# q-optimize/c3

Measured on AMD Instinct MI355X. Metric: full-gate propagators/s, higher is better.
Workload: dtype c128

## Files before the change

c3_amd/csrc/c3p_smalld.hip:

```cpp
#include <type_traits>

#include <cstdlib>
#include "c3p_common.h"
#include "c3p_kernels.h"
#include "c3p_smalld.h"

#ifdef C3P_SMALLD_PART
#define C3P_SMALLD_HAS(p) (C3P_SMALLD_PART == (p))
#else
#define C3P_SMALLD_HAS(p) 1
#endif

extern __shared__ __attribute__((aligned(16))) double c3p_sd_lds[];

namespace {

template <int D>
struct SD {
  static constexpr int NBI = (D + 1) / 2;
  static constexpr int NJ = (D + 3) / 4;
  static constexpr int W = 4 * NJ + 1;
  static constexpr int MAT = 4 * NBI * W;
  static constexpr int IMG = ((MAT - 12 + 31) / 32) * 32 + 12;
};
// ... 575 lines not shown
#pragma unroll
    for (int I = 0; I < NC; ++I)
#pragma unroll
      for (int J = 0; J < NC; ++J) {
        T1[I][J] = Cc.vr[I] * Ur.rc[J];
        T2[I][J] = Sc.vr[I] * Ui.rc[J];
        T3[I][J] = dv[I] * us[J];
      }
  }
  double tr[NC], ti[NC], ar[NC], ai[NC];
#pragma unroll
  for (int J = 0; J < NC; ++J) {
    tr[J] = Cc.vr[0] * Ur.m[0][J];
    ti[J] = Cc.vr[0] * Ui.m[0][J];
#pragma unroll
    for (int K = 1; K < NC; ++K) {
      tr[J] = fma(Cc.vr[K], Ur.m[K][J], tr[J]);
      ti[J] = fma(Cc.vr[K], Ui.m[K][J], ti[J]);
    }
#pragma unroll
    for (int K = 0; K < NC; ++K) {
      tr[J] = fma(Sc.vr[K], Ui.m[K][J], tr[J]);
      ti[J] = fma(-Sc.vr[K], Ur.m[K][J], ti[J]);
    }
    ar[J] = fma(Sc.s, Ui.rc[J], Cc.s * Ur.rc[J]);
    ai[J] = fma(-Sc.s, Ur.rc[J], Cc.s * Ui.rc[J]);
  }
  double Pn[NC];
#pragma unroll
  for (int I = 0; I < NC; ++I) Pn[I] = fma(Sc.vr[I], Qs, Cc.vr[I] * Ub.Ps);
  double ts = Cc.vr[0] * Ub.Pc[0];
#pragma unroll
  for (int K = 1; K < NC; ++K) ts = fma(Cc.vr[K], Ub.Pc[K], ts);
#pragma unroll
  for (int K = 0; K < NC; ++K) ts = fma(Sc.vr[K], Qc[K], ts);
  const double es = fma(Sc.s, Qs, Cc.s * Ub.Ps);
#pragma unroll
  for (int K = 0; K < NC; ++K)
#pragma unroll
    for (int I = 0; I < NC; ++I) {
      Pn[I] = mfma4(Cc.m[K][I], Ub.Pc[K], Pn[I]);
#pragma unroll
      for (int J = 0; J < NC; ++J) {
        T1[I][J] = mfma4(Cc.m[K][I], Ur.m[K][J], T1[I][J]);
        T2[I][J] = mfma4(Sc.m[K][I], Ui.m[K][J], T2[I][J]);
        T3[I][J] = mfma4(Dm[K][I], Us[K][J], T3[I][J]);
      }
      Pn[I] = mfma4(Sc.m[K][I], Qc[K], Pn[I]);
    }
#pragma unroll
  for (int I = 0; I < NC; ++I) {
    Ur.rc[I] = mfma4(1.0, tr[I], ar[I]);
    Ui.rc[I] = mfma4(1.0, ti[I], ai[I]);
  }
  Ub.Ps = mfma4(1.0, ts, es);
#pragma unroll
  for (int I = 0; I < NC; ++I) Ub.Pc[I] = Pn[I];
#pragma unroll
  for (int I = 0; I < NC; ++I)
#pragma unroll
    for (int J = 0; J < NC; ++J) {
      Ur.m[I][J] = T1[I][J] + T2[I][J];
      Ui.m[I][J] = (T3[I][J] - T1[I][J]) + T2[I][J];
    }
}

__device__ __forceinline__ void plan_q4(double nrm, int& r, int& s) {
  const double th[5] = {4.0e-4, 5.45e-2, 3.18e-1, 8.16e-1, 1.49};
  int best_r = 5, best_s = 0, best_cost = 1 << 30;
#pragma unroll
  for (int i = 0; i < 5; ++i) {
    int si = c3p_squarings(nrm, th[i]);
    const int cost = i + si;
    if (cost < best_cost || (cost == best_cost && si <= best_s)) {
      best_cost = cost;
      best_r = i + 1;
      best_s = si;
    }
  }
  r = best_r;
  s = best_s;
}

template <int D>
__device__ __forceinline__ void row_phase_factors(const double* row_phase, const LanePos& lp, double (&pc)[SD<D>::NBI],
                                                  double (&ps)[SD<D>::NBI]) {
#pragma unroll
  for (int I = 0; I < SD<D>::NBI; ++I) {
    const int row = 2 * I + (lp.r >> 1);
    pc[I] = 1.0, ps[I] = 0.0;
    if (row_phase != nullptr && row < D) sincos(row_phase[row], &ps[I], &pc[I]);
  }
}

template <int D>
__device__ __forceinline__ void scale_rows(const double (&zh)[SD<D>::NBI][SD<D>::NJ], const double (&pr)[SD<D>::NBI],
                                           const double (&pi)[SD<D>::NBI], const LanePos& lp,
                                           double (&out)[SD<D>::NBI][SD<D>::NJ]) {
  using C = SD<D>;
  double oth[C::NBI][C::NJ];
#pragma unroll
  for (int I = 0; I < C::NBI; ++I)
#pragma unroll
    for (int J = 0; J < C::NJ; ++J) oth[I][J] = __shfl_xor(zh[I][J], 16);
#pragma unroll
  for (int I = 0; I < C::NBI; ++I)
#pragma unroll
    for (int J = 0; J < C::NJ; ++J)
      out[I][J] = (lp.r & 1) ? fma(pr[I], zh[I][J], pi[I] * oth[I][J]) : fma(pr[I], zh[I][J], -pi[I] * oth[I][J]);
}

template <int D, bool WRITE_THROUGH = false>
__device__ __forceinline__ void store_plain(const double (&zh)[SD<D>::NBI][SD<D>::NJ], double* dst,
                                            double sr, double si, const double* row_phase,
                                            const LanePos& lp, bool active, const double* pre_c = nullptr,
                                            const double* pre_s = nullptr) {
  using C = SD<D>;
  double pr[C::NBI], pi[C::NBI];
#pragma unroll
  for (int I = 0; I < C::NBI; ++I) {
    const int row = 2 * I + (lp.r >> 1);
    pr[I] = sr, pi[I] = si;
    if (pre_c != nullptr) {
      pr[I] = sr * pre_c[I] - si * pre_s[I];
      pi[I] = sr * pre_s[I] + si * pre_c[I];
    } else if (row_phase != nullptr && row < D) {
      double sn, cs;
      sincos(row_phase[row], &sn, &cs);
      pr[I] = sr * cs - si * sn;
      pi[I] = sr * sn + si * cs;
    }
  }
  double outv[C::NBI][C::NJ];
  scale_rows<D>(zh, pr, pi, lp, outv);
#pragma unroll
  for (int I = 0; I < C::NBI; ++I) {
    const int row = 2 * I + (lp.r >> 1);
#pragma unroll
    for (int J = 0; J < C::NJ; ++J) {
      const int col = 4 * J + lp.c;
      if (active && row < D && col < D) {
        double* p = dst + (row * D + col) * 2 + (lp.r & 1);
        if constexpr (WRITE_THROUGH) {
          __hip_atomic_store(reinterpret_cast<unsigned long long*>(p), (unsigned long long)__double_as_longlong(outv[I][J]),
                             __ATOMIC_RELAXED, __HIP_MEMORY_SCOPE_AGENT);
        } else {
          *p = outv[I][J];
        }
      }
    }
  }
}

__device__ __forceinline__ double wave_sum64(double v) {
#pragma unroll
  for (int o = 32; o > 0; o >>= 1) v += __shfl_xor(v, o);
  return v;
}
__device__ __forceinline__ double wave_max64(double v) {
#pragma unroll
  for (int o = 32; o > 0; o >>= 1) v = fmax(v, __shfl_xor(v, o));
  return v;
}

constexpr int SD_CSW = 16;

template <int D>
__device__ __forceinline__ double sd_colsum(const double* g, int j) {
  constexpr int W = SD<D>::W;
  double cs = 0.0;
  if (j < D) {
    double ar[D], ai[D];
#pragma unroll
    for (int i = 0; i < D; ++i) ar[i] = g[(2 * i) * W + j], ai[i] = g[(2 * i + 1) * W + j];
#pragma unroll
    for (int i = 0; i < D; ++i) cs += sqrt(fma(ar[i], ar[i], ai[i] * ai[i]));
  }
  return cs;
}

template <int D>
__device__ __forceinline__ void sd_colsums(const double* tab, int K, double* csb, int lane, int first = 0, int step = 1) {
  constexpr int MAT = SD<D>::MAT;
  for (int t0 = first; t0 <= K; t0 += 4 * step) {
    const int ti = t0 + (lane >> 4) * step;
    if (ti <= K) csb[ti * SD_CSW + (lane & 15)] = sd_colsum<D>(tab + ti * (MAT + 4), lane & 15);
  }
}

template <class F>
__device__ __forceinline__ double c3p_sd_segment_norm(const double* csb, int K, int idx16, F&& maxk) {
  double v = csb[idx16];
  for (int k = 0; k < K; ++k) v = fma(maxk(k), csb[(k + 1) * SD_CSW + idx16], v);
  v = fmax(v, __shfl_xor(v, 1));
  v = fmax(v, __shfl_xor(v, 2));
  v = fmax(v, __shfl_xor(v, 16));
  v = fmax(v, __shfl_xor(v, 32));
  return v;
}

template <int D>
__device__ __forceinline__ void build_tables(const SmallArgs& A, int sample, double* tab, double* csb, int lane, int first = 0, int step = 1) {
  using C = SD<D>;
  constexpr int MAT = C::MAT, W = C::W;
  constexpr int NE = (D * D + 63) / 64;
  for (int ti = first; ti <= A.K; ti += step) {
    double* out = tab + ti * (MAT + 4);
    const cplx* h = (ti == 0) ? A.h0 + (long)sample * A.h0_bstride
                              : A.hks + (long)sample * A.hks_bstride + (long)(ti - 1) * D * D;
    for (int e = lane; e < MAT; e += 64) out[e] = 0.0;
    double gr[NE], gi[NE];
    double tim = 0.0;
#pragma unroll
    for (int q = 0; q < NE; ++q) {
      const int e = lane + 64 * q;
      gr[q] = gi[q] = 0.0;
      if (e < D * D) {
        const cplx x = h[e];
        gr[q] = x.y * A.dt;
        gi[q] = -x.x * A.dt;
        if (e / D == e % D) tim += gi[q];
      }
    }
    const double mur = 0.0, mui = wave_sum64(tim) / D;
    wave_sync();
    double remax = 0.0;
#pragma unroll
    for (int q = 0; q < NE; ++q) {
      const int e = lane + 64 * q;
      if (e < D * D) {
        const int i = e / D, j = e - i * D;
        if (i == j) {
          gr[q] -= mur;
          gi[q] -= mui;
        }
        out[(2 * i) * W + j] = gr[q];
        out[(2 * i + 1) * W + j] = gi[q];
        remax = fmax(remax, fabs(gr[q]));
      }
    }
    wave_sync();
    const double cs = sd_colsum<D>(out, lane);
    if (lane < SD_CSW) csb[ti * SD_CSW + lane] = cs;
    const double nrm = wave_max64(cs);
    double asym = 0.0, rsk = 0.0;
#pragma unroll
    for (int q = 0; q < NE; ++q) {
      const int e = lane + 64 * q;
      if (e < D * D) {
        const int i = e / D, j = e - i * D;
        asym = fmax(asym, fabs(gi[q] - out[(2 * j + 1) * W + i]));
        rsk = fmax(rsk, fabs(gr[q] + out[(2 * j) * W + i]));
      }
    }
    asym = wave_max64(asym);
    rsk = wave_max64(rsk);
    if (asym > 1e-14 * nrm) remax = fmax(remax, asym);
    remax = wave_max64(remax);
    if (remax > 0.0 && fmax(asym, rsk) <= 1e-14 * nrm) remax = -remax;
    if (lane == 0) {
      out[MAT + 0] = mur;
      out[MAT + 1] = mui;
      out[MAT + 2] = nrm;
      out[MAT + 3] = remax;
    }
  }
  wave_sync();
}

template <int D, bool GIVEN, bool DUS, bool XG = false, bool MW = false, bool SPLIT = false>
__global__ void __launch_bounds__((MW ? 512 : 64), 2) smalld_chain_kernel(SmallArgs A) {
  using C = SD<D>;
  constexpr int NBI = C::NBI, NJ = C::NJ, W = C::W, MAT = C::MAT, IMG = C::IMG;
  const int lane = MW ? (threadIdx.x & 63) : threadIdx.x;
  const int wv = MW ? __builtin_amdgcn_readfirstlane(threadIdx.x >> 6) : 0;
  const int nwv = MW ? (int)(blockDim.x >> 6) : 1;
#ifdef C3P_SD_TIMING
  long long tk0 = wall_clock64(), tk1 = 0, tk2 = 0, tk3 = 0, tk4 = 0, tk5 = 0, tk6 = 0, tk7 = 0, tk8 = 0, tk9 = 0, tkl = 0, tka = 0, tkb = 0;
#define SD_TICK(v) v = wall_clock64()
#else
#define SD_TICK(v)
#endif
  LanePos lp;
  lp.r = lane >> 4;
  lp.b = (lane >> 2) & 3;
  lp.c = lane & 3;
  lp.idx16 = lp.r * 4 + lp.c;
  const int K = A.K;
  double* tab = c3p_sd_lds;
  const int SG = ((K + ((SPLIT && K > 0) ? 1 : 0)) * A.Lmax) | 1;
  double* img = tab + ((GIVEN || XG) ? 0 : (1 + K) * (MAT + 4)) + wv * (4 * IMG + 4 * SG);
  double* sg = img + 4 * IMG;
  double* csb = (!MW && (1 + K) * SD_CSW <= 4 * IMG) ? img : tab + (1 + K) * (MAT + 4) + nwv * (4 * IMG + 4 * SG);

  long lblock = blockIdx.x;
  if constexpr (MW)
    lblock = (long)blockIdx.x * nwv + wv;
  else if ((gridDim.x & 7) == 0)
    lblock = (long)(blockIdx.x & 7) * (gridDim.x >> 3) + (blockIdx.x >> 3);
  const long chain = lblock * 4 + lp.b;
  const long nchains = (long)A.B * A.S;
  const bool valid = chain < nchains;
  const long cc = valid ? chain : nchains - 1;
  const int sample = (int)(cc / A.S);
  const int seg = (int)(cc - (long)sample * A.S);
  int n0 = (int)(((long)seg * A.N) / A.S);
  int n1 = (int)(((long)(seg + 1) * A.N) / A.S);
  int len, tmax;
  auto split_segments = [&](int seg_long) {
    if (MW && seg_long > 0) {
      const int h = A.S >> 1;
      const long rest = (long)A.N - (long)h * seg_long;
      n0 = seg < h ? seg * seg_long : h * seg_long + (int)(((long)(seg - h) * rest) / h);
      n1 = seg + 1 <= h ? (seg + 1) * seg_long : h * seg_long + (int)(((long)(seg + 1 - h) * rest) / h);
    }
    len = n1 - n0;
    tmax = A.Lmax;
    if (MW && seg_long > 0) {
      int m = len;
      m = max(m, __shfl_xor(m, 4));
      m = max(m, __shfl_xor(m, 8));
      tmax = __builtin_amdgcn_readfirstlane(m);
    }
  };
  split_segments(A.seg_long);

  const int woff = lp.b * IMG + lp.r * W + lp.c;
  const int roff = lp.b * IMG + (2 * (lp.c >> 1) + ((lp.c ^ lp.r) & 1)) * W + (lp.r >> 1);
  const unsigned negmask = (((lp.c & 1) == 0) && ((lp.r & 1) == 1)) ? 0x80000000u : 0u;
  const int toff = lp.r * W + lp.c;
  const int ddelta = (lp.r & 1) ? 1000 : ((lp.r >> 1) - lp.c);
  const int rhalf = lp.r >> 1;

  double U[NBI][NJ];
  double mus_r = 0.0, mus_i = 0.0;
  bool img_holds_U = false;

  if constexpr (GIVEN) {
    const double* base = reinterpret_cast<const double*>(A.mats) + ((long)sample * A.N + n0) * D * D * 2;
    for (int t = 0; t < tmax; ++t) {
      const bool act = valid && t < len;
      double P[NBI][NJ];
      const double* src = base + (long)(act ? t : 0) * D * D * 2;
#pragma unroll
      for (int I = 0; I < NBI; ++I)
#pragma unroll
        for (int J = 0; J < NJ; ++J) {
          const int row = 2 * I + (lp.r >> 1), col = 4 * J + lp.c;
          P[I][J] = (act && row < D && col < D) ? src[(row * D + col) * 2 + (lp.r & 1)] : 0.0;
        }
      if (t == 0) {
#pragma unroll
        for (int I = 0; I < NBI; ++I)
#pragma unroll
          for (int J = 0; J < NJ; ++J) U[I][J] = P[I][J];
      } else {
        double acc[NBI][NJ];
#pragma unroll
        for (int I = 0; I < NBI; ++I)
#pragma unroll
          for (int J = 0; J < NJ; ++J) acc[I][J] = 0.0;
        if (A.right_order) {
          write_image<D>(U, img, woff);
          mm_img<D>(img, roff, negmask, P, acc);
        } else {
          write_image<D>(P, img, woff);
          mm_img<D>(img, roff, negmask, U, acc);
        }
#pragma unroll
        for (int I = 0; I < NBI; ++I)
#pragma unroll
          for (int J = 0; J < NJ; ++J) U[I][J] = act ? acc[I][J] : U[I][J];
      }
    }
  } else {
    double nrm = 0.0;
    if constexpr (XG) {
      const double* mt = A.meta + ((long)sample * A.N + n0) * 4;
      for (int t = lp.idx16; t < A.Lmax; t += 16)
        if (valid && t < len) nrm = fmax(nrm, mt[(long)t * 4 + 2]);
      nrm = fmax(nrm, __shfl_xor(nrm, 1));
      nrm = fmax(nrm, __shfl_xor(nrm, 2));
      nrm = fmax(nrm, __shfl_xor(nrm, 16));
      nrm = fmax(nrm, __shfl_xor(nrm, 32));
    } else {
    constexpr int PF_K = 2, PF_T = 3;
    const bool prefetch = MW && A.inline_tables && K <= PF_K && A.Lmax <= 16 * PF_T;
    double pre[PF_K][PF_T];
    if (prefetch) {
#pragma unroll
      for (int k = 0; k < PF_K; ++k)
#pragma unroll
        for (int i = 0; i < PF_T; ++i) {
          const int t = lp.idx16 + 16 * i;
          const double* sk = A.signals + ((long)sample * K + (k < K ? k : 0)) * A.N + n0;
          pre[k][i] = (k < K && valid && t < len) ? sk[t] : 0.0;
        }
    }
    if (A.inline_tables) {
      build_tables<D>(A, __builtin_amdgcn_readfirstlane(sample), tab, csb, lane, wv, nwv);
    } else {
      const double* gt0 = A.tables + (long)(A.tab_per_sample ? sample : 0) * (1 + K) * (MAT + 4);
      for (int e = (MW ? (int)threadIdx.x : lane); e < (1 + K) * (MAT + 4); e += 64 * nwv) tab[e] = gt0[e];
      __syncthreads();
      sd_colsums<D>(tab, K, csb, lane, wv, nwv);
    }
    if constexpr (!MW) __syncthreads();
    auto seg_max = [&](int k, bool from_lds) {
      const double* s = A.signals + ((long)sample * K + k) * A.N + n0;
      double cmax = 0.0;
      for (int t = lp.idx16; t < A.Lmax; t += 16) {
        double v;
        if (from_lds) {
          v = sg[lp.b * SG + k * A.Lmax + t];
        } else {
          v = (valid && t < len) ? s[t] : 0.0;
          sg[lp.b * SG + k * A.Lmax + t] = v;
        }
        cmax = fmax(cmax, fabs(v));
      }
      cmax = fmax(cmax, __shfl_xor(cmax, 1));
      cmax = fmax(cmax, __shfl_xor(cmax, 2));
      cmax = fmax(cmax, __shfl_xor(cmax, 16));
      cmax = fmax(cmax, __shfl_xor(cmax, 32));
      return cmax;
    };
    SD_TICK(tk8);
    if constexpr (MW) {
      if (prefetch) {
#pragma unroll
        for (int k = 0; k < PF_K; ++k)
#pragma unroll
          for (int i = 0; i < PF_T; ++i) {
            const int t = lp.idx16 + 16 * i;
            if (k < K && t < A.Lmax) sg[lp.b * SG + k * A.Lmax + t] = pre[k][i];
          }
      } else {
        for (int k = 0; k < K; ++k) (void)seg_max(k, false);
      }
      SD_TICK(tk9);
      __syncthreads();
      if (A.seg_long_c > 0 && A.seg_long_c != A.seg_long) {
        bool re = (A.mode == C3P_MODE_UNITARY);
        for (int k = 0; k <= K; ++k) re = re && (tab[k * (MAT + 4) + MAT + 3] == 0.0);
        if (__builtin_amdgcn_readfirstlane((int)re) == 0) {
          wave_sync();
          split_segments(A.seg_long_c);
          for (int k = 0; k < K; ++k) (void)seg_max(k, false);
          wave_sync();
        }
      }
    }
    nrm = c3p_sd_segment_norm(csb, K, lp.idx16, [&](int k) { return seg_max(k, MW); });
    }
    nrm = fmax(nrm, __shfl_xor(nrm, 4));
    nrm = fmax(nrm, __shfl_xor(nrm, 8));
    nrm = readfirstlane_f64(nrm);
    bool realH = !XG && (A.mode == C3P_MODE_UNITARY);
    if constexpr (!XG)
      for (int k = 0; k <= K; ++k) realH = realH && (tab[k * (MAT + 4) + MAT + 3] == 0.0);
    realH = __builtin_amdgcn_readfirstlane((int)realH) != 0;
    MfmaPlan plan = {0, 0, 0};
    int t18n = 0;
    if (!realH) {
      bool normalG = !XG && (A.mode == C3P_MODE_UNITARY) && !(A.no_t18n & 1);
      if constexpr (!XG)
        for (int k = 0; k <= K; ++k) normalG = normalG && (tab[k * (MAT + 4) + MAT + 3] <= 0.0);
      t18n = __builtin_amdgcn_readfirstlane((int)normalG);
      plan = c3p_pick_plan_mfma(nrm, t18n ? C3P_T18N_THETA : C3P_T18_THETA, t18n != 0 && !(A.no_t18n & 2));
    }
    const int pr = __builtin_amdgcn_readfirstlane(plan.r);
    const int ps = __builtin_amdgcn_readfirstlane(plan.s);
    const int t18 = __builtin_amdgcn_readfirstlane(plan.t18);
    const double scale = ldexp(1.0, -ps);
    __syncthreads();
    SD_TICK(tk1);

    if (realH) {
      constexpr int NB = RD<D>::NB;
      typedef double RMat[NB][NB];
      const int ps_r = __builtin_amdgcn_readfirstlane(c3p_squarings(nrm, C3P_MM8_THETA));
      const double rscale = ldexp(1.0, -ps_r);
      const int swap_lane = 16 * lp.c + 4 * lp.b + lp.r;
      const int tail_lane = 16 * lp.c + 4 * lp.b;
      const int row0_lane = 4 * lp.b + lp.c;
      RMat Ur, Ui;
      int yo[NB];
      double ymask[NB];
#pragma unroll
      for (int I = 0; I < NB; ++I) {
        const bool ok = 4 * I + lp.r < D;
        yo[I] = (2 * (ok ? 4 * I + lp.r : 0) + 1) * W + lp.c;
        ymask[I] = ok ? 1.0 : 0.0;
      }
      if constexpr (SPLIT) {
        static_assert(!SPLIT || (D % 4 == 1 && D > 4 && !DUS), "core + border form: D = 5, 9 without slice output");
        constexpr int NC = (D - 1) / 4;
        typedef SMat<NC> SM;
        GMat<NC> Gr, Gi;
        GBorder<NC> Gb;
        int so[NC], sro[NC], sco[NC];
#pragma unroll
        for (int I = 0; I < NC; ++I) {
          so[I] = (2 * (4 * I + lp.r) + 1) * W + lp.c;
          sro[I] = (2 * (4 * I + lp.r) + 1) * W + (D - 1);
          sco[I] = (2 * (4 * I + lp.c) + 1) * W + (D - 1);
        }
        constexpr int sso = (2 * (D - 1) + 1) * W + (D - 1);
        const bool deg6 = __builtin_amdgcn_readfirstlane((int)(nrm * rscale <= C3P_MM6_THETA)) != 0;
        {
          double ph = 0.0;
          for (int k = 0; k < K; ++k) {
            const double mk = tab[(k + 1) * (MAT + 4) + MAT + 1];
            for (int t = lp.idx16; t < A.Lmax; t += 16) {
              const double c0 = sg[lp.b * SG + k * A.Lmax + t];
              ph = c3p_phase_add(ph, c0 * mk);
              sg[lp.b * SG + k * A.Lmax + t] = -rscale * c0;
            }
          }
          if (K > 0)
            for (int t = lp.idx16; t < A.Lmax; t += 16) sg[lp.b * SG + K * A.Lmax + t] = (valid && t < len) ? -rscale : 0.0;
          ph = c3p_phase_add(ph, __shfl_xor(ph, 1));
          ph = c3p_phase_add(ph, __shfl_xor(ph, 2));
          ph = c3p_phase_add(ph, __shfl_xor(ph, 16));
          ph = c3p_phase_add(ph, __shfl_xor(ph, 32));
          mus_i = c3p_phase_add(ph, (double)(valid ? len : 0) * c3p_phase_add(0.0, tab[MAT + 1]));
          wave_sync();
        }
        int tfast = valid ? len : 0;
        tfast = min(tfast, __shfl_xor(tfast, 4));
        tfast = min(tfast, __shfl_xor(tfast, 8));
        tfast = min(__builtin_amdgcn_readfirstlane(tfast), tmax);
        auto slice_exp = [&](int t, auto deg6_tag, auto k_tag, auto weighted_tag, auto sq_tag, bool vc, SM& Cm, SM& acc) {
          constexpr bool DEG6 = decltype(deg6_tag)::value;
          constexpr int KC = decltype(k_tag)::value;
          constexpr bool WEIGHTED = decltype(weighted_tag)::value, SQ = decltype(sq_tag)::value;
          static_assert(WEIGHTED || (KC >= 0 && !SQ), "the unweighted drift is the form of compile-time K without squarings");
          const double* ap = sg + lp.b * SG;
          SM Y;
          if constexpr (WEIGHTED) {
            const double a0 = (KC == 0 || (KC < 0 && K == 0)) ? ((valid && t < len) ? -rscale : 0.0) : ap[K * A.Lmax + t];
#pragma unroll
            for (int I = 0; I < NC; ++I) {
#pragma unroll
              for (int J = 0; J < NC; ++J) Y.m[I][J] = a0 * lds_ld(tab + so[I] + J * 4);
              Y.vr[I] = a0 * lds_ld(tab + sro[I]);
              Y.vc[I] = a0 * lds_ld(tab + sco[I]);
            }
            Y.s = a0 * lds_ld(tab + sso);
          } else if constexpr (KC == 0) {
#pragma unroll
            for (int I = 0; I < NC; ++I) {
#pragma unroll
              for (int J = 0; J < NC; ++J) Y.m[I][J] = -lds_ld(tab + so[I] + J * 4);
              Y.vr[I] = -lds_ld(tab + sro[I]);
              Y.vc[I] = -lds_ld(tab + sco[I]);
            }
            Y.s = -lds_ld(tab + sso);
          } else {
            const double a1 = ap[t];
            const double* t1 = tab + (MAT + 4);
#pragma unroll
            for (int I = 0; I < NC; ++I) {
#pragma unroll
              for (int J = 0; J < NC; ++J) Y.m[I][J] = fma(a1, lds_ld(t1 + so[I] + J * 4), -lds_ld(tab + so[I] + J * 4));
              Y.vr[I] = fma(a1, lds_ld(t1 + sro[I]), -lds_ld(tab + sro[I]));
              Y.vc[I] = fma(a1, lds_ld(t1 + sco[I]), -lds_ld(tab + sco[I]));
            }
            Y.s = fma(a1, lds_ld(t1 + sso), -lds_ld(tab + sso));
          }
          auto add_table = [&](int k) {
            const double ak = ap[k * A.Lmax + t];
            const double* tk = tab + (k + 1) * (MAT + 4);
#pragma unroll
            for (int I = 0; I < NC; ++I) {
#pragma unroll
              for (int J = 0; J < NC; ++J) Y.m[I][J] = fma(ak, lds_ld(tk + so[I] + J * 4), Y.m[I][J]);
              Y.vr[I] = fma(ak, lds_ld(tk + sro[I]), Y.vr[I]);
              Y.vc[I] = fma(ak, lds_ld(tk + sco[I]), Y.vc[I]);
            }
            Y.s = fma(ak, lds_ld(tk + sso), Y.s);
          };
          if constexpr (KC >= 0) {
#pragma unroll
            for (int k = WEIGHTED ? 0 : 1; k < KC; ++k) add_table(k);
          } else {
            for (int k = 0; k < K; ++k) add_table(k);
          }
          SM W1, W2, W3, Sp, acs;
          s8_zero(W1), s8_zero(W2), s8_zero(W3);
          mm_s8(Y, Y, W1);
          s8_finish(W1, swap_lane, tail_lane);
          mm_s8(W1, W1, W2);
          s8_finish(W2, swap_lane, tail_lane);
          if constexpr (DEG6) {
            mm_s8(W1, W2, W3);
            s8_finish(W3, swap_lane, tail_lane);
            s8_comb<NC, true, true>(acc, c3p_mm6_cos[3], c3p_mm6_cos[4], c3p_mm6_cos[5], c3p_mm6_cos[6], W1, W2, W3, lp);
            s8_comb<NC, true, true>(acs, c3p_mm6_sinc[3], c3p_mm6_sinc[4], c3p_mm6_sinc[5], c3p_mm6_sinc[6], W1, W2, W3, lp);
            s8_finish_lower(acc, swap_lane);
            s8_finish_lower(acs, swap_lane);
            s8_comb<NC, false, true>(Cm, c3p_mm6_cos[0], c3p_mm6_cos[1], c3p_mm6_cos[2], 0.0, W1, W2, W3, lp);
            s8_comb<NC, false, true>(Sp, c3p_mm6_sinc[0], c3p_mm6_sinc[1], c3p_mm6_sinc[2], 0.0, W1, W2, W3, lp);
            mm_s8x2r(acc, acs, W3, Cm, Sp);
          } else {
            SM W4;
            s8_zero(W4);
            mm_s8(W1, W2, W3);
            mm_s8(W2, W2, W4);
            s8_finish(W4, swap_lane, tail_lane);
            s8_comb<NC, true, true>(acc, c3p_mm8_cos[4], c3p_mm8_cos[5], c3p_mm8_cos[6], c3p_mm8_cos[7], W1, W2, W3, lp);
            s8_comb<NC, true, true>(acs, c3p_mm8_sinc[4], c3p_mm8_sinc[5], c3p_mm8_sinc[6], c3p_mm8_sinc[7], W1, W2, W3, lp);
#pragma unroll
            for (int I = 0; I < NC; ++I) {
#pragma unroll
              for (int J = I; J < NC; ++J) {
                acc.m[I][J] = fma(c3p_mm8_cos[8], W4.m[I][J], acc.m[I][J]);
                acs.m[I][J] = fma(c3p_mm8_sinc[8], W4.m[I][J], acs.m[I][J]);
              }
              acc.vr[I] = fma(c3p_mm8_cos[8], W4.vr[I], acc.vr[I]);
              acs.vr[I] = fma(c3p_mm8_sinc[8], W4.vr[I], acs.vr[I]);
            }
            acc.s = fma(c3p_mm8_cos[8], W4.s, acc.s);
            acs.s = fma(c3p_mm8_sinc[8], W4.s, acs.s);
            s8_finish_lower(acc, swap_lane);
            s8_finish_lower(acs, swap_lane);
            s8_comb<NC, true, true>(Cm, c3p_mm8_cos[0], c3p_mm8_cos[1], c3p_mm8_cos[2], c3p_mm8_cos[3], W1, W2, W3, lp);
            s8_comb<NC, true, true>(Sp, c3p_mm8_sinc[0], c3p_mm8_sinc[1], c3p_mm8_sinc[2], c3p_mm8_sinc[3], W1, W2, W3, lp);
            mm_s8x2r(acc, acs, W4, Cm, Sp);
          }
          s8_finish_lower(Cm, swap_lane);
          s8_finish_lower(Sp, swap_lane);
          s8_zero(acc);
          mm_s8(Sp, Y, acc);
          s8_finish_lower(acc, swap_lane);
          if (vc) {
            s8_finish_vc(Cm, tail_lane);
            s8_finish_vc(acc, tail_lane);
          }
          if constexpr (SQ) {
            for (int it = 0; it < ps_r; ++it) {
              SM Dm, Sm, C2, SC;
#pragma unroll
              for (int I = 0; I < NC; ++I) {
#pragma unroll
                for (int J = 0; J < NC; ++J) {
                  Dm.m[I][J] = Cm.m[I][J] - acc.m[I][J];
                  Sm.m[I][J] = Cm.m[I][J] + acc.m[I][J];
                }
                Dm.vr[I] = Cm.vr[I] - acc.vr[I];
                Sm.vr[I] = Cm.vr[I] + acc.vr[I];
                Dm.vc[I] = Cm.vc[I] - acc.vc[I];
                Sm.vc[I] = Cm.vc[I] + acc.vc[I];
              }
              Dm.s = Cm.s - acc.s;
              Sm.s = Cm.s + acc.s;
              s8_zero(C2), s8_zero(SC);
              mm_s8(Dm, Sm, C2);
              mm_s8(acc, Cm, SC);
#pragma unroll
              for (int I = 0; I < NC; ++I) {
#pragma unroll
                for (int J = I; J < NC; ++J) {
                  Cm.m[I][J] = C2.m[I][J];
                  acc.m[I][J] = 2.0 * SC.m[I][J];
                }
                Cm.vr[I] = C2.vr[I];
                acc.vr[I] = 2.0 * SC.vr[I];
              }
              Cm.s = C2.s;
              acc.s = 2.0 * SC.s;
              s8_finish(Cm, swap_lane, tail_lane);
              s8_finish(acc, swap_lane, tail_lane);
            }
          }
        };
        auto step_loop = [&](int t0, int t1, auto deg6_tag, auto k_tag, auto weighted_tag, auto sq_tag, bool vc) {
          for (int t = t0; t < t1; ++t) {
            SM Cm, acc;
            slice_exp(t, deg6_tag, k_tag, weighted_tag, sq_tag, vc, Cm, acc);
            chain_step8(Cm, acc, Gr, Gi, Gb);
          }
        };
        auto split_loop_k = [&](auto deg6_tag) {
// ... 328 lines not shown
          write_image<D>(L, img, woff);
#pragma unroll
          for (int I = 0; I < NBI; ++I)
#pragma unroll
            for (int J = 0; J < NJ; ++J) {
              R[I][J] = fma(c3p_e4n[4], A2[I][J], A3[I][J]);
              y1[I][J] = fma(c3p_e4n[5], A3[I][J], c3p_e4n[6] * A2[I][J]);
            }
          mm_img<D>(img, roff, negmask, R, y1);
        }
        {
          double L[NBI][NJ], R[NBI][NJ];
#pragma unroll
          for (int I = 0; I < NBI; ++I)
#pragma unroll
            for (int J = 0; J < NJ; ++J) L[I][J] = fma(c3p_e4n[7], A2[I][J], fma(c3p_e4n[8], X[I][J], y1[I][J]));
          write_image<D>(L, img, woff);
#pragma unroll
          for (int I = 0; I < NBI; ++I)
#pragma unroll
            for (int J = 0; J < NJ; ++J) {
              R[I][J] = fma(c3p_e4n[9], A3[I][J], fma(c3p_e4n[10], X[I][J], y1[I][J]));
              double v = fma(c3p_e4n[11], y1[I][J], c3p_e4n[12] * A3[I][J]);
              v = fma(c3p_e4n[13], A2[I][J], v);
              v = fma(c3p_e4n[14], X[I][J], v);
              if (2 * I - 4 * J >= -1 && 2 * I - 4 * J <= 3) {
                const bool on = (ddelta == 4 * J - 2 * I) && (2 * I + rhalf < D);
                v += on ? c3p_e4n[15] : 0.0;
              }
              P[I][J] = v;
            }
          mm_img<D>(img, roff, negmask, R, P);
        }
      } else {
      mm_img<D>(img, roff, negmask, A2, A3);
      if constexpr (T18) {
        double A6[NBI][NJ];
#pragma unroll
        for (int I = 0; I < NBI; ++I)
#pragma unroll
          for (int J = 0; J < NJ; ++J) A6[I][J] = 0.0;
        write_image<D>(A3, img, woff);
        mm_img<D>(img, roff, negmask, A3, A6);
        double acc[NBI][NJ];
        {
          double B1[NBI][NJ], B5[NBI][NJ];
          lincomb6<D>(B1, 0.0, t18_a11, t18_a21, t18_a31, 0.0, X, A2, A3, A6, ddelta, rhalf);
          write_image<D>(B1, img, woff);
          lincomb6<D>(B5, 0.0, 0.0, t18_b24, t18_b34, t18_b64, X, A2, A3, A6, ddelta, rhalf);
          lincomb6<D>(acc, t18_b03, t18_b13, t18_b23, t18_b33, t18_b63, X, A2, A3, A6, ddelta, rhalf);
          mm_img<D>(img, roff, negmask, B5, acc);
        }
        {
          double L[NBI][NJ];
          lincomb6<D>(L, t18_b02, t18_b12, t18_b22, t18_b32, t18_b62, X, A2, A3, A6, ddelta, rhalf);
#pragma unroll
          for (int I = 0; I < NBI; ++I)
#pragma unroll
            for (int J = 0; J < NJ; ++J) L[I][J] += acc[I][J];
          write_image<D>(L, img, woff);
        }
        lincomb6<D>(P, 0.0, t18_b11, t18_b21, t18_b31, t18_b61, X, A2, A3, A6, ddelta, rhalf);
        mm_img<D>(img, roff, negmask, acc, P);
      } else {
        {
          double A4[NBI][NJ];
  #pragma unroll
          for (int I = 0; I < NBI; ++I)
  #pragma unroll
            for (int J = 0; J < NJ; ++J) A4[I][J] = 0.0;
          mm_img<D>(img, roff, negmask, A3, A4);
          const int j = pr - 1;
          poly_block<D>(P, c3p_inv_fact[4 * j], c3p_inv_fact[4 * j + 1], c3p_inv_fact[4 * j + 2],
                        c3p_inv_fact[4 * j + 3], X, A2, A3, ddelta, rhalf);
          const double cm = c3p_inv_fact[4 * pr];
  #pragma unroll
          for (int I = 0; I < NBI; ++I)
  #pragma unroll
            for (int J = 0; J < NJ; ++J) P[I][J] = fma(cm, A4[I][J], P[I][J]);
          if (pr > 1) write_image<D>(A4, img, woff);
        }
        for (int j = pr - 2; j >= 0; --j) {
          double acc[NBI][NJ];
          poly_block<D>(acc, c3p_inv_fact[4 * j], c3p_inv_fact[4 * j + 1], c3p_inv_fact[4 * j + 2],
                        c3p_inv_fact[4 * j + 3], X, A2, A3, ddelta, rhalf);
          mm_img<D>(img, roff, negmask, P, acc);
  #pragma unroll
          for (int I = 0; I < NBI; ++I)
  #pragma unroll
            for (int J = 0; J < NJ; ++J) P[I][J] = acc[I][J];
        }
      }
      }
      for (int it = 0; it < ps; ++it) {
        write_image<D>(P, img, woff);
        double acc[NBI][NJ];
#pragma unroll
        for (int I = 0; I < NBI; ++I)
#pragma unroll
          for (int J = 0; J < NJ; ++J) acc[I][J] = 0.0;
        mm_img<D>(img, roff, negmask, P, acc);
        const bool sq = !XG || it < my_s;
#pragma unroll
        for (int I = 0; I < NBI; ++I)
#pragma unroll
          for (int J = 0; J < NJ; ++J) P[I][J] = sq ? acc[I][J] : P[I][J];
      }
      if constexpr (DUS) {
        double sn, cs;
        sincos(mu_i, &sn, &cs);
        const double er = exp(mu_r);
        double* dst = reinterpret_cast<double*>(A.dUs_out) + ((long)sample * A.N + n0 + (act ? t : 0)) * D * D * 2;
        store_plain<D>(P, dst, er * cs, er * sn, nullptr, lp, act);
      }
      if (t == 0) {
#pragma unroll
        for (int I = 0; I < NBI; ++I)
#pragma unroll
          for (int J = 0; J < NJ; ++J) U[I][J] = P[I][J];
        mus_r = mu_r;
        mus_i = c3p_phase_add(0.0, mu_i);
      } else {
        write_image<D>(P, img, woff);
        double acc[NBI][NJ];
#pragma unroll
        for (int I = 0; I < NBI; ++I)
#pragma unroll
          for (int J = 0; J < NJ; ++J) acc[I][J] = 0.0;
        mm_img<D>(img, roff, negmask, U, acc);
#pragma unroll
        for (int I = 0; I < NBI; ++I)
#pragma unroll
          for (int J = 0; J < NJ; ++J) U[I][J] = acc[I][J];
        mus_r += mu_r;
        mus_i = c3p_phase_add(mus_i, mu_i);
      }
    }
    };
    if (t18 == 2)
      complex_loop(std::integral_constant<int, 2>{});
    else if (t18)
      complex_loop(std::integral_constant<int, 1>{});
    else
      complex_loop(std::integral_constant<int, 0>{});
    }
  }
  SD_TICK(tk2);
#ifdef C3P_SD_TIMING
  if (tkl == 0) tkl = tk2;
#endif
  if constexpr (!GIVEN) {
    if (A.fuse) {
      double tr = mus_r, ti = mus_i;
      tr += __shfl_xor(tr, 4);
      tr += __shfl_xor(tr, 8);
      ti = c3p_phase_add(ti, __shfl_xor(ti, 4));
      ti = c3p_phase_add(ti, __shfl_xor(ti, 8));
      const int rrest = roff - lp.b * IMG;
      double V[NBI][NJ], Wt[NBI][NJ];
      constexpr bool FOLD_SPLIT = MW && NBI * NJ > 2 && D <= 9;
      auto fold_slots = [&](const double (&M)[NBI][NJ], bool in_image) {
        if (!in_image) write_image<D>(M, img, woff);
        if constexpr (FOLD_SPLIT) {
          const int wrest = woff - lp.b * IMG;
          mm_split<D, 2>(img + ((lp.b & 2) + 1) * IMG + rrest, img + (lp.b & 2) * IMG + wrest, negmask, lp.b & 1);
          mm_split<D, 4>(img + 2 * IMG + rrest, img + wrest, negmask, lp.b);
#pragma unroll
          for (int I = 0; I < NBI; ++I)
#pragma unroll
            for (int J = 0; J < NJ; ++J) Wt[I][J] = img[wrest + I * 4 * W + J * 4];
        } else {
          const int roff1 = ((lp.b + 1) & 3) * IMG + rrest;
          const int roff2 = ((lp.b + 2) & 3) * IMG + rrest;
#pragma unroll
          for (int I = 0; I < NBI; ++I)
#pragma unroll
            for (int J = 0; J < NJ; ++J) V[I][J] = Wt[I][J] = 0.0;
          mm_img<D>(img, roff1, negmask, M, V);
          write_image<D>(V, img, woff);
          mm_img<D>(img, roff2, negmask, V, Wt);
        }
      };
      fold_slots(U, img_holds_U);
      SD_TICK(tka);
      const int nW = A.S >> 2;
      const int wq = seg >> 2;
      const double* ph = A.fr_phase ? A.fr_phase + (long)sample * D : nullptr;
      double* dst = reinterpret_cast<double*>(A.final_out) + (long)sample * D * D * 2;
      const int lo = (lp.b * nW) >> 2, hi = ((lp.b + 1) * nW) >> 2;
      const int cnt = hi - lo;
      const int cmax = (nW + 3) >> 2;
      double sn, cs;
      sincos(ti, &sn, &cs);
      double er = 1.0;
      if (__ballot(tr != 0.0) != 0) er = exp(tr);
      SD_TICK(tkb);
      if constexpr (MW) {
        {
          double pr[NBI], pi[NBI];
#pragma unroll
          for (int I = 0; I < NBI; ++I) pr[I] = er * cs, pi[I] = er * sn;
          scale_rows<D>(Wt, pr, pi, lp, V);
        }
        write_image<D>(V, img, woff);
        SD_TICK(tk3);
        double phc[NBI], phs[NBI];
        if (wv == 0) row_phase_factors<D>(ph, lp, phc, phs);
        __syncthreads();
#ifdef C3P_SD_TIMING
        if (blockIdx.x == 7 && lane == 0)
          printf("sd wave %d: slices %d, prologue to the table barrier %lld, behind it %lld, loop ends at %lld (100 MHz ticks after the wave's start); "
                 "layout %lld products %lld phase %lld partial store %lld\n", wv, tmax, tk9 - tk0, tk1 - tk9, tkl - tk0, tk2 - tkl, tka - tk2, tkb - tka, tk3 - tkb);
#endif
        if (wv != 0) return;
        SD_TICK(tk5);
        const int pstride = 4 * IMG + 4 * SG;
        const int woff0 = woff - lp.b * IMG;
#pragma unroll
        for (int I = 0; I < NBI; ++I)
#pragma unroll
          for (int J = 0; J < NJ; ++J) {
            const int row = 2 * I + (lp.r >> 1), col = 4 * J + lp.c;
            const double idv = (row < D && row == col && (lp.r & 1) == 0) ? 1.0 : 0.0;
            U[I][J] = cnt > 0 ? img[lo * pstride + woff0 + I * 4 * W + J * 4] : idv;
          }
        for (int t = 1; t < cmax; ++t) {
          const bool act = t < cnt;
          double acc[NBI][NJ];
#pragma unroll
          for (int I = 0; I < NBI; ++I)
#pragma unroll
            for (int J = 0; J < NJ; ++J) acc[I][J] = 0.0;
          mm_img<D>(img, (act ? lo + t : 0) * pstride + rrest, negmask, U, acc);
#pragma unroll
          for (int I = 0; I < NBI; ++I)
#pragma unroll
            for (int J = 0; J < NJ; ++J) U[I][J] = act ? acc[I][J] : U[I][J];
        }
        SD_TICK(tk6);
        fold_slots(U, false);
        SD_TICK(tk7);
        store_plain<D>(Wt, dst, 1.0, 0.0, ph, lp, lp.b == 0, phc, phs);
#ifdef C3P_SD_TIMING
        SD_TICK(tk4);
        if (blockIdx.x == 0 && threadIdx.x == 0)
          printf("sd timing (100 MHz ticks): tables %lld signals %lld prologue %lld loop %lld fold4+store %lld barrier %lld level1 %lld fold2 %lld store %lld total %lld\n", tk8 - tk0, tk9 - tk8, tk1 - tk0, tk2 - tk1, tk3 - tk2, tk5 - tk3, tk6 - tk5, tk7 - tk6, tk4 - tk7, tk4 - tk0);
#endif
        return;
      }
      if (nW == 1) {
        store_plain<D>(Wt, dst, er * cs, er * sn, ph, lp, valid && lp.b == 0);
        return;
      }
      {
        double* pdst = reinterpret_cast<double*>(A.seg_out) + ((long)sample * nW + wq) * D * D * 2;
        store_plain<D, true>(Wt, pdst, er * cs, er * sn, nullptr, lp, valid && lp.b == 0);
      }
      asm volatile("s_waitcnt vmcnt(0)" ::: "memory");
      int old = 0;
      if (lane == 0)
        old = __hip_atomic_fetch_add(A.counters + sample, 1, __ATOMIC_RELAXED, __HIP_MEMORY_SCOPE_AGENT);
      old = __builtin_amdgcn_readfirstlane(old);
      if (old != nW - 1) return;
      if (lane == 0) A.counters[sample] = 0;
      __builtin_amdgcn_fence(__ATOMIC_ACQUIRE, "agent");
      const double* base = reinterpret_cast<const double*>(A.seg_out) + ((long)sample * nW + lo) * D * D * 2;
      double Pn[NBI][NJ];
      auto fetch = [&](double (&P)[NBI][NJ], int t) {
        const bool act = t < cnt;
        const double* src = base + (long)(act ? t : 0) * D * D * 2;
#pragma unroll
        for (int I = 0; I < NBI; ++I)
#pragma unroll
          for (int J = 0; J < NJ; ++J) {
            const int row = 2 * I + (lp.r >> 1), col = 4 * J + lp.c;
            const bool in = row < D && col < D;
            const double idv = (in && row == col && (lp.r & 1) == 0) ? 1.0 : 0.0;
            P[I][J] = (act && in) ? src[(row * D + col) * 2 + (lp.r & 1)] : idv;
          }
      };
      fetch(U, 0);
      if (cmax > 1) fetch(Pn, 1);
      for (int t = 1; t < cmax; ++t) {
        double P[NBI][NJ];
#pragma unroll
        for (int I = 0; I < NBI; ++I)
#pragma unroll
          for (int J = 0; J < NJ; ++J) P[I][J] = Pn[I][J];
        if (t + 1 < cmax) fetch(Pn, t + 1);
        {
          double acc[NBI][NJ];
#pragma unroll
          for (int I = 0; I < NBI; ++I)
#pragma unroll
            for (int J = 0; J < NJ; ++J) acc[I][J] = 0.0;
          write_image<D>(P, img, woff);
          mm_img<D>(img, roff, negmask, U, acc);
#pragma unroll
          for (int I = 0; I < NBI; ++I)
#pragma unroll
            for (int J = 0; J < NJ; ++J) U[I][J] = acc[I][J];
        }
      }
      fold_slots(U, false);
      store_plain<D>(Wt, dst, 1.0, 0.0, ph, lp, lp.b == 0);
      return;
    }
  }
  double sn, cs;
  sincos(mus_i, &sn, &cs);
// ... 1226 lines not shown
```

Measured before the change: 2.898 million.

## Use DPP/permlane reductions, overlap table build with amplitude loads, simplify MW indexing

Replaces ds_bpermute-based shuffles in the wave reductions with DPP row operations and permlane16/32 swaps, and batches several max-reductions into one interleaved pass. Global loads of Hamiltonian entries are issued before the table build, and the MW amplitude fetch with its max computation is moved under those loads so per-segment maxima stay in registers. MW chain indexing now uses shifts, which assumes S is a power of two. A barrier is dropped for MW and the realH/normalG flag scans are merged. This adds hardware-specific intrinsics and a power-of-two assumption that could break other shapes.

```diff
diff --git a/c3_amd/csrc/c3p_smalld.hip b/c3_amd/csrc/c3p_smalld.hip
--- a/c3_amd/csrc/c3p_smalld.hip
+++ b/c3_amd/csrc/c3p_smalld.hip
@@ -751,15 +751,66 @@
   }
 }
 
+template <int CTRL>
+__device__ __forceinline__ double dpp_f64(double v) {
+  int lo = __double2loint(v), hi = __double2hiint(v);
+  lo = __builtin_amdgcn_mov_dpp(lo, CTRL, 0xf, 0xf, true);
+  hi = __builtin_amdgcn_mov_dpp(hi, CTRL, 0xf, 0xf, true);
+  return __hiloint2double(hi, lo);
+}
+constexpr int DPP_XOR1 = 0xB1, DPP_XOR2 = 0x4E, DPP_XOR3 = 0x1B;
+constexpr int DPP_HALF_MIRROR = 0x141;
+constexpr int DPP_ROR1 = 0x121, DPP_ROR2 = 0x122, DPP_ROR4 = 0x124, DPP_ROR8 = 0x128;
+__device__ __forceinline__ void pair_xor16(double v, double& a, double& b) {
+  const unsigned lo = __double2loint(v), hi = __double2hiint(v);
+  const auto rl = __builtin_amdgcn_permlane16_swap(lo, lo, false, false);
+  const auto rh = __builtin_amdgcn_permlane16_swap(hi, hi, false, false);
+  a = __hiloint2double(rh[0], rl[0]);
+  b = __hiloint2double(rh[1], rl[1]);
+}
+__device__ __forceinline__ void pair_xor32(double v, double& a, double& b) {
+  const unsigned lo = __double2loint(v), hi = __double2hiint(v);
+  const auto rl = __builtin_amdgcn_permlane32_swap(lo, lo, false, false);
+  const auto rh = __builtin_amdgcn_permlane32_swap(hi, hi, false, false);
+  a = __hiloint2double(rh[0], rl[0]);
+  b = __hiloint2double(rh[1], rl[1]);
+}
+__device__ __forceinline__ double rows_max(double v) {
+  double a, b;
+  pair_xor16(v, a, b);
+  v = fmax(a, b);
+  pair_xor32(v, a, b);
+  return fmax(a, b);
+}
 __device__ __forceinline__ double wave_sum64(double v) {
-#pragma unroll
-  for (int o = 32; o > 0; o >>= 1) v += __shfl_xor(v, o);
+  double a, b;
+  pair_xor32(v, a, b);
+  v = a + b;
+  pair_xor16(v, a, b);
+  v = a + b;
+  v += dpp_f64<DPP_ROR8>(v);
+  v += dpp_f64<DPP_ROR4>(v);
+  v += dpp_f64<DPP_XOR2>(v);
+  v += dpp_f64<DPP_XOR1>(v);
   return v;
 }
-__device__ __forceinline__ double wave_max64(double v) {
-#pragma unroll
-  for (int o = 32; o > 0; o >>= 1) v = fmax(v, __shfl_xor(v, o));
-  return v;
+template <int N>
+__device__ __forceinline__ void wave_max64(double (&v)[N]) {
+#pragma unroll
+  for (int n = 0; n < N; ++n) v[n] = fmax(v[n], dpp_f64<DPP_ROR1>(v[n]));
+#pragma unroll
+  for (int n = 0; n < N; ++n) v[n] = fmax(v[n], dpp_f64<DPP_ROR2>(v[n]));
+#pragma unroll
+  for (int n = 0; n < N; ++n) v[n] = fmax(v[n], dpp_f64<DPP_ROR4>(v[n]));
+#pragma unroll
+  for (int n = 0; n < N; ++n) v[n] = fmax(v[n], dpp_f64<DPP_ROR8>(v[n]));
+#pragma unroll
+  for (int n = 0; n < N; ++n) v[n] = rows_max(v[n]);
+}
+__device__ __forceinline__ double chain_max16(double v) {
+  v = fmax(v, dpp_f64<DPP_XOR1>(v));
+  v = fmax(v, dpp_f64<DPP_XOR2>(v));
+  return rows_max(v);
 }
 
 constexpr int SD_CSW = 16;
@@ -788,9 +839,14 @@
 }
 
 template <class F>
-__device__ __forceinline__ double c3p_sd_segment_norm(const double* csb, int K, int idx16, F&& maxk) {
+__device__ __forceinline__ double c3p_sd_segment_col(const double* csb, int K, int idx16, F&& maxk) {
   double v = csb[idx16];
   for (int k = 0; k < K; ++k) v = fma(maxk(k), csb[(k + 1) * SD_CSW + idx16], v);
+  return v;
+}
+template <class F>
+__device__ __forceinline__ double c3p_sd_segment_norm(const double* csb, int K, int idx16, F&& maxk) {
+  double v = c3p_sd_segment_col(csb, K, idx16, maxk);
   v = fmax(v, __shfl_xor(v, 1));
   v = fmax(v, __shfl_xor(v, 2));
   v = fmax(v, __shfl_xor(v, 16));
@@ -798,28 +854,32 @@
   return v;
 }
 
-template <int D>
-__device__ __forceinline__ void build_tables(const SmallArgs& A, int sample, double* tab, double* csb, int lane, int first = 0, int step = 1) {
+template <int D, class F>
+__device__ __forceinline__ void build_tables(const SmallArgs& A, int sample, double* tab, double* csb, int lane, int first, int step,
+                                             F&& under_loads) {
+#pragma clang fp contract(off)
   using C = SD<D>;
   constexpr int MAT = C::MAT, W = C::W;
   constexpr int NE = (D * D + 63) / 64;
+  if (first > A.K) under_loads();
   for (int ti = first; ti <= A.K; ti += step) {
     double* out = tab + ti * (MAT + 4);
     const cplx* h = (ti == 0) ? A.h0 + (long)sample * A.h0_bstride
                               : A.hks + (long)sample * A.hks_bstride + (long)(ti - 1) * D * D;
+    cplx x[NE];
+#pragma unroll
+    for (int q = 0; q < NE; ++q) x[q] = h[min(lane + 64 * q, D * D - 1)];
+    if (ti == first) under_loads();
     for (int e = lane; e < MAT; e += 64) out[e] = 0.0;
     double gr[NE], gi[NE];
     double tim = 0.0;
 #pragma unroll
     for (int q = 0; q < NE; ++q) {
       const int e = lane + 64 * q;
-      gr[q] = gi[q] = 0.0;
-      if (e < D * D) {
-        const cplx x = h[e];
-        gr[q] = x.y * A.dt;
-        gi[q] = -x.x * A.dt;
-        if (e / D == e % D) tim += gi[q];
-      }
+      const bool in = e < D * D;
+      gr[q] = in ? x[q].y * A.dt : 0.0;
+      gi[q] = in ? -x[q].x * A.dt : 0.0;
+      if (in && e / D == e % D) tim += gi[q];
     }
     const double mur = 0.0, mui = wave_sum64(tim) / D;
     wave_sync();
@@ -841,7 +901,6 @@
     wave_sync();
     const double cs = sd_colsum<D>(out, lane);
     if (lane < SD_CSW) csb[ti * SD_CSW + lane] = cs;
-    const double nrm = wave_max64(cs);
     double asym = 0.0, rsk = 0.0;
 #pragma unroll
     for (int q = 0; q < NE; ++q) {
@@ -852,10 +911,11 @@
         rsk = fmax(rsk, fabs(gr[q] + out[(2 * j) * W + i]));
       }
     }
-    asym = wave_max64(asym);
-    rsk = wave_max64(rsk);
+    double red[4] = {cs, asym, rsk, remax};
+    wave_max64(red);
+    const double nrm = red[0];
+    asym = red[1], rsk = red[2], remax = red[3];
     if (asym > 1e-14 * nrm) remax = fmax(remax, asym);
-    remax = wave_max64(remax);
     if (remax > 0.0 && fmax(asym, rsk) <= 1e-14 * nrm) remax = -remax;
     if (lane == 0) {
       out[MAT + 0] = mur;
@@ -892,33 +952,43 @@
   double* sg = img + 4 * IMG;
   double* csb = (!MW && (1 + K) * SD_CSW <= 4 * IMG) ? img : tab + (1 + K) * (MAT + 4) + nwv * (4 * IMG + 4 * SG);
 
-  long lblock = blockIdx.x;
-  if constexpr (MW)
-    lblock = (long)blockIdx.x * nwv + wv;
-  else if ((gridDim.x & 7) == 0)
-    lblock = (long)(blockIdx.x & 7) * (gridDim.x >> 3) + (blockIdx.x >> 3);
-  const long chain = lblock * 4 + lp.b;
-  const long nchains = (long)A.B * A.S;
-  const bool valid = chain < nchains;
-  const long cc = valid ? chain : nchains - 1;
-  const int sample = (int)(cc / A.S);
-  const int seg = (int)(cc - (long)sample * A.S);
-  int n0 = (int)(((long)seg * A.N) / A.S);
-  int n1 = (int)(((long)(seg + 1) * A.N) / A.S);
+  long cc;
+  int sample, seg, n0, n1;
+  bool valid;
+  const int sshift = 31 - __clz(A.S);
+  if constexpr (MW) {
+    valid = true;
+    sample = blockIdx.x;
+    seg = 4 * wv + lp.b;
+    cc = (long)sample * A.S + seg;
+    n0 = (int)(((long)seg * A.N) >> sshift);
+    n1 = (int)(((long)(seg + 1) * A.N) >> sshift);
+  } else {
+    long lblock = blockIdx.x;
+    if ((gridDim.x & 7) == 0) lblock = (long)(blockIdx.x & 7) * (gridDim.x >> 3) + (blockIdx.x >> 3);
+    const long chain = lblock * 4 + lp.b;
+    const long nchains = (long)A.B * A.S;
+    valid = chain < nchains;
+    cc = valid ? chain : nchains - 1;
+    sample = (int)(cc / A.S);
+    seg = (int)(cc - (long)sample * A.S);
+    n0 = (int)(((long)seg * A.N) / A.S);
+    n1 = (int)(((long)(seg + 1) * A.N) / A.S);
+  }
   int len, tmax;
   auto split_segments = [&](int seg_long) {
     if (MW && seg_long > 0) {
       const int h = A.S >> 1;
       const long rest = (long)A.N - (long)h * seg_long;
-      n0 = seg < h ? seg * seg_long : h * seg_long + (int)(((long)(seg - h) * rest) / h);
-      n1 = seg + 1 <= h ? (seg + 1) * seg_long : h * seg_long + (int)(((long)(seg + 1 - h) * rest) / h);
+      n0 = seg < h ? seg * seg_long : h * seg_long + (int)(((long)(seg - h) * rest) >> (sshift - 1));
+      n1 = seg + 1 <= h ? (seg + 1) * seg_long : h * seg_long + (int)(((long)(seg + 1 - h) * rest) >> (sshift - 1));
     }
     len = n1 - n0;
     tmax = A.Lmax;
     if (MW && seg_long > 0) {
       int m = len;
-      m = max(m, __shfl_xor(m, 4));
-      m = max(m, __shfl_xor(m, 8));
+      m = max(m, __builtin_amdgcn_mov_dpp(m, DPP_ROR4, 0xf, 0xf, true));
+      m = max(m, __builtin_amdgcn_mov_dpp(m, DPP_ROR8, 0xf, 0xf, true));
       tmax = __builtin_amdgcn_readfirstlane(m);
     }
   };
@@ -974,6 +1044,7 @@
     }
   } else {
     double nrm = 0.0;
+    bool realH = false, normalG = false;
     if constexpr (XG) {
       const double* mt = A.meta + ((long)sample * A.N + n0) * 4;
       for (int t = lp.idx16; t < A.Lmax; t += 16)
@@ -982,6 +1053,8 @@
       nrm = fmax(nrm, __shfl_xor(nrm, 2));
       nrm = fmax(nrm, __shfl_xor(nrm, 16));
       nrm = fmax(nrm, __shfl_xor(nrm, 32));
+      nrm = fmax(nrm, __shfl_xor(nrm, 4));
+      nrm = fmax(nrm, __shfl_xor(nrm, 8));
     } else {
     constexpr int PF_K = 2, PF_T = 3;
     const bool prefetch = MW && A.inline_tables && K <= PF_K && A.Lmax <= 16 * PF_T;
@@ -996,15 +1069,10 @@
           pre[k][i] = (k < K && valid && t < len) ? sk[t] : 0.0;
         }
     }
-    if (A.inline_tables) {
-      build_tables<D>(A, __builtin_amdgcn_readfirstlane(sample), tab, csb, lane, wv, nwv);
-    } else {
-      const double* gt0 = A.tables + (long)(A.tab_per_sample ? sample : 0) * (1 + K) * (MAT + 4);
-      for (int e = (MW ? (int)threadIdx.x : lane); e < (1 + K) * (MAT + 4); e += 64 * nwv) tab[e] = gt0[e];
-      __syncthreads();
-      sd_colsums<D>(tab, K, csb, lane, wv, nwv);
-    }
-    if constexpr (!MW) __syncthreads();
+    double cm[PF_K];
+#pragma unroll
+    for (int k = 0; k < PF_K; ++k) cm[k] = 0.0;
+    const bool cm_regs = MW && K <= PF_K;
     auto seg_max = [&](int k, bool from_lds) {
       const double* s = A.signals + ((long)sample * K + k) * A.N + n0;
       double cmax = 0.0;
@@ -1018,53 +1086,80 @@
         }
         cmax = fmax(cmax, fabs(v));
       }
-      cmax = fmax(cmax, __shfl_xor(cmax, 1));
-      cmax = fmax(cmax, __shfl_xor(cmax, 2));
-      cmax = fmax(cmax, __shfl_xor(cmax, 16));
-      cmax = fmax(cmax, __shfl_xor(cmax, 32));
-      return cmax;
+      return chain_max16(cmax);
     };
-    SD_TICK(tk8);
-    if constexpr (MW) {
+    auto keep_max = [&](int k, double m) {
+#pragma unroll
+      for (int q = 0; q < PF_K; ++q)
+        if (k == q) cm[q] = m;
+    };
+    auto fetch_amplitudes = [&]() {
       if (prefetch) {
 #pragma unroll
-        for (int k = 0; k < PF_K; ++k)
+        for (int k = 0; k < PF_K; ++k) {
+          double m = 0.0;
 #pragma unroll
           for (int i = 0; i < PF_T; ++i) {
             const int t = lp.idx16 + 16 * i;
             if (k < K && t < A.Lmax) sg[lp.b * SG + k * A.Lmax + t] = pre[k][i];
+            m = fmax(m, fabs(pre[k][i]));
           }
+          cm[k] = chain_max16(m);
+        }
       } else {
-        for (int k = 0; k < K; ++k) (void)seg_max(k, false);
-      }
-      SD_TICK(tk9);
+        for (int k = 0; k < K; ++k) keep_max(k, seg_max(k, false));
+      }
+    };
+    if (A.inline_tables) {
+      build_tables<D>(A, __builtin_amdgcn_readfirstlane(sample), tab, csb, lane, wv, nwv, [&]() {
+        if constexpr (MW) fetch_amplitudes();
+      });
+    } else {
+      const double* gt0 = A.tables + (long)(A.tab_per_sample ? sample : 0) * (1 + K) * (MAT + 4);
+      for (int e = (MW ? (int)threadIdx.x : lane); e < (1 + K) * (MAT + 4); e += 64 * nwv) tab[e] = gt0[e];
+      if constexpr (MW) fetch_amplitudes();
       __syncthreads();
-      if (A.seg_long_c > 0 && A.seg_long_c != A.seg_long) {
-        bool re = (A.mode == C3P_MODE_UNITARY);
-        for (int k = 0; k <= K; ++k) re = re && (tab[k * (MAT + 4) + MAT + 3] == 0.0);
-        if (__builtin_amdgcn_readfirstlane((int)re) == 0) {
-          wave_sync();
-          split_segments(A.seg_long_c);
-          for (int k = 0; k < K; ++k) (void)seg_max(k, false);
-          wave_sync();
-        }
-      }
-    }
-    nrm = c3p_sd_segment_norm(csb, K, lp.idx16, [&](int k) { return seg_max(k, MW); });
-    }
-    nrm = fmax(nrm, __shfl_xor(nrm, 4));
-    nrm = fmax(nrm, __shfl_xor(nrm, 8));
+      sd_colsums<D>(tab, K, csb, lane, wv, nwv);
+    }
+    SD_TICK(tk8);
+    SD_TICK(tk9);
+    __syncthreads();
+    bool all_real = true, all_normal = true;
+    {
+      double f[PF_K + 1];
+#pragma unroll
+      for (int q = 0; q <= PF_K; ++q) f[q] = tab[min(q, K) * (MAT + 4) + MAT + 3];
+#pragma unroll
+      for (int q = 0; q <= PF_K; ++q) all_real = all_real & (f[q] == 0.0), all_normal = all_normal & (f[q] <= 0.0);
+      for (int k = PF_K + 1; k <= K; ++k) {
+        const double fk = tab[k * (MAT + 4) + MAT + 3];
+        all_real = all_real & (fk == 0.0), all_normal = all_normal & (fk <= 0.0);
+      }
+    }
+    realH = __builtin_amdgcn_readfirstlane((int)((A.mode == C3P_MODE_UNITARY) && all_real)) != 0;
+    normalG = (A.mode == C3P_MODE_UNITARY) && !(A.no_t18n & 1) && all_normal;
+    if constexpr (MW) {
+      if (A.seg_long_c > 0 && A.seg_long_c != A.seg_long && !realH) {
+        wave_sync();
+        split_segments(A.seg_long_c);
+        for (int k = 0; k < K; ++k) keep_max(k, seg_max(k, false));
+        wave_sync();
+      }
+    }
+    {
+      double col[1] = {c3p_sd_segment_col(csb, K, lp.idx16, [&](int k) {
+        static_assert(PF_K == 2, "the select below reads cm[0] and cm[1]");
+        if (cm_regs) return k == 0 ? cm[0] : cm[1];
+        return seg_max(k, MW);
+      })};
+      wave_max64(col);
+      nrm = col[0];
+    }
+    }
     nrm = readfirstlane_f64(nrm);
-    bool realH = !XG && (A.mode == C3P_MODE_UNITARY);
-    if constexpr (!XG)
-      for (int k = 0; k <= K; ++k) realH = realH && (tab[k * (MAT + 4) + MAT + 3] == 0.0);
-    realH = __builtin_amdgcn_readfirstlane((int)realH) != 0;
     MfmaPlan plan = {0, 0, 0};
     int t18n = 0;
     if (!realH) {
-      bool normalG = !XG && (A.mode == C3P_MODE_UNITARY) && !(A.no_t18n & 1);
-      if constexpr (!XG)
-        for (int k = 0; k <= K; ++k) normalG = normalG && (tab[k * (MAT + 4) + MAT + 3] <= 0.0);
       t18n = __builtin_amdgcn_readfirstlane((int)normalG);
       plan = c3p_pick_plan_mfma(nrm, t18n ? C3P_T18N_THETA : C3P_T18_THETA, t18n != 0 && !(A.no_t18n & 2));
     }
@@ -1072,7 +1167,7 @@
     const int ps = __builtin_amdgcn_readfirstlane(plan.s);
     const int t18 = __builtin_amdgcn_readfirstlane(plan.t18);
     const double scale = ldexp(1.0, -ps);
-    __syncthreads();
+    if constexpr (!MW) __syncthreads();
     SD_TICK(tk1);
 
     if (realH) {
@@ -1119,16 +1214,19 @@
           }
           if (K > 0)
             for (int t = lp.idx16; t < A.Lmax; t += 16) sg[lp.b * SG + K * A.Lmax + t] = (valid && t < len) ? -rscale : 0.0;
-          ph = c3p_phase_add(ph, __shfl_xor(ph, 1));
-          ph = c3p_phase_add(ph, __shfl_xor(ph, 2));
-          ph = c3p_phase_add(ph, __shfl_xor(ph, 16));
-          ph = c3p_phase_add(ph, __shfl_xor(ph, 32));
+          double pa, pb;
+          ph = c3p_phase_add(ph, dpp_f64<DPP_XOR1>(ph));
+          ph = c3p_phase_add(ph, dpp_f64<DPP_XOR2>(ph));
+          pair_xor16(ph, pa, pb);
+          ph = c3p_phase_add(pa, pb);
+          pair_xor32(ph, pa, pb);
+          ph = c3p_phase_add(pa, pb);
           mus_i = c3p_phase_add(ph, (double)(valid ? len : 0) * c3p_phase_add(0.0, tab[MAT + 1]));
           wave_sync();
         }
         int tfast = valid ? len : 0;
-        tfast = min(tfast, __shfl_xor(tfast, 4));
-        tfast = min(tfast, __shfl_xor(tfast, 8));
+        tfast = min(tfast, __builtin_amdgcn_mov_dpp(tfast, DPP_ROR4, 0xf, 0xf, true));
+        tfast = min(tfast, __builtin_amdgcn_mov_dpp(tfast, DPP_ROR8, 0xf, 0xf, true));
         tfast = min(__builtin_amdgcn_readfirstlane(tfast), tmax);
         auto slice_exp = [&](int t, auto deg6_tag, auto k_tag, auto weighted_tag, auto sq_tag, bool vc, SM& Cm, SM& acc) {
           constexpr bool DEG6 = decltype(deg6_tag)::value;
@@ -1763,10 +1861,10 @@
   if constexpr (!GIVEN) {
     if (A.fuse) {
       double tr = mus_r, ti = mus_i;
-      tr += __shfl_xor(tr, 4);
-      tr += __shfl_xor(tr, 8);
-      ti = c3p_phase_add(ti, __shfl_xor(ti, 4));
-      ti = c3p_phase_add(ti, __shfl_xor(ti, 8));
+      tr += dpp_f64<DPP_HALF_MIRROR>(dpp_f64<DPP_XOR3>(tr));
+      tr += dpp_f64<DPP_ROR8>(tr);
+      ti = c3p_phase_add(ti, dpp_f64<DPP_HALF_MIRROR>(dpp_f64<DPP_XOR3>(ti)));
+      ti = c3p_phase_add(ti, dpp_f64<DPP_ROR8>(ti));
       const int rrest = roff - lp.b * IMG;
       double V[NBI][NJ], Wt[NBI][NJ];
       constexpr bool FOLD_SPLIT = MW && NBI * NJ > 2 && D <= 9;
```

After: 2.998 million, median of 6. 1.03x the previous value.
